# aws-samples/sample-s3-hybrid-cache

Hardware: AMD Instinct MI355X
Metric: LZ4 encode+decode GiB/s (device-resident), 64 KiB blocks, 1/2/4/8 GPU (higher is better)
Workload: dtype u8

## Files before the change

### sample-s3-hybrid-cache_amd/csrc/s3hc_kernels.hip

```cpp
#include <hip/hip_runtime.h>
#include <stdint.h>

#include "s3hc_plan.hpp"
#include "s3hc_knobs.hpp"
#include "s3hc_lz4.h"

namespace s3hc {

__device__ __forceinline__ uint32_t rotl32(uint32_t x, int r) {
    return __builtin_amdgcn_alignbit(x, x, 32 - r);
}
__device__ __forceinline__ uint32_t rdl(uint32_t v, uint32_t l) {
    return (uint32_t)__builtin_amdgcn_readlane((int)v, (int)l);
}
__device__ __forceinline__ int lane_id() { return __builtin_amdgcn_mbcnt_hi(~0u, __builtin_amdgcn_mbcnt_lo(~0u, 0)); }

#ifndef S3HC_WALK_PRIO
#define S3HC_WALK_PRIO 3
#endif
#define WALK_PRIO_ON() __builtin_amdgcn_s_setprio(S3HC_WALK_PRIO)
#define WALK_PRIO_OFF() __builtin_amdgcn_s_setprio(0)

__device__ __forceinline__ void wave_sync() {
    __builtin_amdgcn_fence(__ATOMIC_RELEASE, "wavefront");
    __builtin_amdgcn_wave_barrier();
    __builtin_amdgcn_fence(__ATOMIC_ACQUIRE, "wavefront");
}

#if defined(S3HC_DIAG_LEVEL) && S3HC_DIAG_LEVEL == 10
#define S3HC_PROF 1
__device__ unsigned long long g_prof[32];
#define PROF_NOW() __builtin_amdgcn_s_memtime()
#define PROF_ADD(arr, k, v) (arr)[k] += (v)
#else
#define PROF_NOW() 0ull
#define PROF_ADD(arr, k, v) ((void)(v))
#endif

__device__ __forceinline__ uint32_t lds32u(const uint8_t* lds, uint32_t i) {
    const uint32_t* w = (const uint32_t*)(lds + (i & ~3u));
    return __builtin_amdgcn_alignbyte(w[1], w[0], i & 3u);
}

__device__ __forceinline__ uint32_t gld32u(const uint8_t* p, uint32_t avail) {
    uintptr_t a = (uintptr_t)p;
    const uint32_t* w = (const uint32_t*)(a & ~(uintptr_t)3);
    uint32_t sh = (uint32_t)(a & 3);
    uint32_t lo = w[0];
    uint32_t hi = (sh != 0 && avail > 4 - sh) ? w[1] : 0u;
    return __builtin_amdgcn_alignbyte(hi, lo, sh);
}

template <int CTRL, int ROWMASK>
__device__ __forceinline__ uint32_t dpp0(uint32_t x) {
    return (uint32_t)__builtin_amdgcn_update_dpp(0, (int)x, CTRL, ROWMASK, 0xF, false);
}
__device__ __forceinline__ uint32_t wave_incl_sum(uint32_t x) {
    x += dpp0<0x111, 0xF>(x);
    x += dpp0<0x112, 0xF>(x);
    x += dpp0<0x114, 0xF>(x);
    x += dpp0<0x118, 0xF>(x);
    x += dpp0<0x142, 0xA>(x);
    x += dpp0<0x143, 0xC>(x);
    return x;
}
__device__ __forceinline__ uint32_t umax32(uint32_t a, uint32_t b) { return a > b ? a : b; }
__device__ __forceinline__ uint32_t umin32(uint32_t a, uint32_t b) { return a < b ? a : b; }
__device__ __forceinline__ uint32_t wave_incl_max(uint32_t x) {
    x = umax32(x, dpp0<0x111, 0xF>(x));
    x = umax32(x, dpp0<0x112, 0xF>(x));
    x = umax32(x, dpp0<0x114, 0xF>(x));
    x = umax32(x, dpp0<0x118, 0xF>(x));
    x = umax32(x, dpp0<0x142, 0xA>(x));
    x = umax32(x, dpp0<0x143, 0xC>(x));
    return x;
}
__device__ __forceinline__ uint32_t wave_excl_scan(uint32_t v, int) { return wave_incl_sum(v) - v; }
template <int CTRL, int ROWMASK>
__device__ __forceinline__ uint64_t dpp0_64(uint64_t x) {
    return (uint64_t)dpp0<CTRL, ROWMASK>((uint32_t)(x >> 32)) << 32 | dpp0<CTRL, ROWMASK>((uint32_t)x);
}
__device__ __forceinline__ uint64_t wave_incl_sum64(uint64_t x) {
    x += dpp0_64<0x111, 0xF>(x);
    x += dpp0_64<0x112, 0xF>(x);
    x += dpp0_64<0x114, 0xF>(x);
    x += dpp0_64<0x118, 0xF>(x);
    x += dpp0_64<0x142, 0xA>(x);
    x += dpp0_64<0x143, 0xC>(x);
    return x;
}

__device__ void wave_copy_global(uint8_t* dst, const uint8_t* src, uint32_t n, int lane) {
    uintptr_t da = (uintptr_t)dst;
    uint32_t head = (uint32_t)((16 - (da & 15)) & 15);
    if (head > n) head = n;
    if ((uint32_t)lane < head) dst[lane] = src[lane];
    const uint32_t nv = (n - head) >> 4;
    const uint8_t* s = src + head;
    uint8_t* d = dst + head;
    const uintptr_t sa = (uintptr_t)s;
    const uint32_t sh = (uint32_t)(sa & 3);
    const uint32_t* sw = (const uint32_t*)(sa & ~(uintptr_t)3);
    for (uint32_t base = 0; base < nv; base += 64 * 2) {
        const uint32_t ja = base + lane, jb = base + lane + 64;
        const uint32_t ka = ja < nv ? ja : nv - 1, kb = jb < nv ? jb : nv - 1;
        uint4 va, vb;
        if (sh == 0) {
            va = make_uint4(sw[4 * ka], sw[4 * ka + 1], sw[4 * ka + 2], sw[4 * ka + 3]);
            vb = make_uint4(sw[4 * kb], sw[4 * kb + 1], sw[4 * kb + 2], sw[4 * kb + 3]);
        } else {
            const uint32_t a0 = sw[4 * ka], a1 = sw[4 * ka + 1], a2 = sw[4 * ka + 2], a3 = sw[4 * ka + 3], a4 = sw[4 * ka + 4];
            const uint32_t b0 = sw[4 * kb], b1 = sw[4 * kb + 1], b2 = sw[4 * kb + 2], b3 = sw[4 * kb + 3], b4 = sw[4 * kb + 4];
            va = make_uint4(__builtin_amdgcn_alignbyte(a1, a0, sh), __builtin_amdgcn_alignbyte(a2, a1, sh),
                            __builtin_amdgcn_alignbyte(a3, a2, sh), __builtin_amdgcn_alignbyte(a4, a3, sh));
            vb = make_uint4(__builtin_amdgcn_alignbyte(b1, b0, sh), __builtin_amdgcn_alignbyte(b2, b1, sh),
                            __builtin_amdgcn_alignbyte(b3, b2, sh), __builtin_amdgcn_alignbyte(b4, b3, sh));
        }
        if (ja < nv) *(uint4*)(d + 16 * ja) = va;
        if (jb < nv) *(uint4*)(d + 16 * jb) = vb;
    }
    for (uint32_t t = head + 16 * nv + (uint32_t)lane; t < n; t += 64) dst[t] = src[t];
}

__device__ void wave_store_from_lds(uint8_t* dst, const uint8_t* lds, uint32_t n, int lane) {
    uintptr_t da = (uintptr_t)dst;
    uint32_t head = (uint32_t)((16 - (da & 15)) & 15);
    if (head > n) head = n;
    if ((uint32_t)lane < head) dst[lane] = lds[lane];
    uint32_t body = (n - head) & ~15u;
    for (uint32_t c = (uint32_t)lane * 16; c < body; c += 64 * 16) {
        uint32_t i = head + c;
        uint4 v = make_uint4(lds32u(lds, i), lds32u(lds, i + 4), lds32u(lds, i + 8), lds32u(lds, i + 12));
        *(uint4*)(dst + i) = v;
    }
    for (uint32_t t = head + body + (uint32_t)lane; t < n; t += 64) dst[t] = lds[t];
}

#define XP1 2654435761U
#define XP2 2246822519U
#define XP3 3266489917U
#define XP4 668265263U
#define XP5 374761393U

__device__ __forceinline__ uint32_t xround(uint32_t acc, uint32_t in) {
    acc += in * XP2;
    acc = rotl32(acc, 13);
    return acc * XP1;
}

template <uint32_t kIF, bool kPipe>
__device__ __forceinline__ uint32_t xxh32_lanes(const uint8_t* __restrict__ p, uint32_t L, bool act, uint32_t a) {
    const int lane = lane_id();
    const uint32_t ns = L >> 4;
    uint32_t acc = a == 0 ? XP1 + XP2 : (a == 1 ? XP2 : (a == 2 ? 0u : 0u - XP1));
    const uint8_t* q = p + 4 * a;
    uint32_t s = 0;
    if (kPipe && (((uintptr_t)p) & 3) == 0) {
        const uint32_t* w = (const uint32_t*)q;
        uint32_t b0[kIF], b1[kIF], b2[kIF];
        const uint32_t nbt = ns / kIF;
#define XLD(buf, bidx)                                                        \
    {                                                                         \
        const uint32_t bb_ = (bidx) < nbt ? (bidx) : 0u;                      \
        _Pragma("unroll") for (uint32_t k = 0; k < kIF; ++k) buf[k] = w[4 * (bb_ * kIF + k)]; \
    }
#define XUSE(buf) _Pragma("unroll") for (uint32_t k = 0; k < kIF; ++k) acc = xround(acc, buf[k]);
        XLD(b0, 0u)
        XLD(b1, 1u)
        for (uint32_t b = 0; b < nbt; b += 3) {
            XLD(b2, b + 2)
            XUSE(b0)
            XLD(b0, b + 3)
            if (b + 1 < nbt) { XUSE(b1) }
            XLD(b1, b + 4)
            if (b + 2 < nbt) { XUSE(b2) }
        }
#undef XLD
#undef XUSE
        for (s = nbt * kIF; s < ns; ++s) acc = xround(acc, w[4 * s]);
    } else if ((((uintptr_t)p) & 3) == 0) {
        const uint32_t* w = (const uint32_t*)q;
        for (; s + kIF <= ns; s += kIF) {
            uint32_t v[kIF];
#pragma unroll
            for (uint32_t k = 0; k < kIF; ++k) v[k] = w[4 * (s + k)];
#pragma unroll
            for (uint32_t k = 0; k < kIF; ++k) acc = xround(acc, v[k]);
        }
        for (; s < ns; ++s) acc = xround(acc, w[4 * s]);
// ... 1021 lines not shown
                    if (tll > limit - produced) st = S3HC_CORRUPT;
                    else if (tll > cap - produced) st = S3HC_DST_TOO_SMALL;
                    else if (tail == 1) {
                        const uint32_t have = produced + tll;
                        if (toff == 0 || toff > have + hist) st = S3HC_CORRUPT;
                        else if (tml > limit - have) st = S3HC_CORRUPT;
                        else if (tml > cap - have) st = S3HC_DST_TOO_SMALL;
                    }
                    if (st != S3HC_OK) { finish_block(st); continue; }
                    upos += tll + (tail == 1 ? tml : 0u);
                    blk_done = tail == 2;
                }
                if (n == 0 && tail == 0) {
                    if (blk_done) finish_block(S3HC_OK);
                    else q = cur;
                    continue;
                }
                cmd = dpe::C_WIN;
                emit_lo = n ? q + mis : 0xFFFFFFFFu;
                if (lane == 0) {
                    sl.S = S;
                    sl.n = n;
                    sl.ptr = (uint64_t)(uintptr_t)in;
                    sl.tail = tail;
                    sl.tlit = tlit;
                    sl.tll = tll;
                    sl.toff = toff;
                    sl.tml = tml;
                }
                if (blk_done) finish_block(S3HC_OK);
                else q = cur;
            }
            if (lane == 0) sl.cmd = cmd;
            prev_lo = emit_lo;
        } else if (it > 0) {
            const Slot& sl = slots[(it - 1u) & 1u];
            auto rfl = [](uint32_t v) -> uint32_t { return (uint32_t)__builtin_amdgcn_readfirstlane((int)v); };
            const uint32_t cmd = rfl(sl.cmd);
            const uint8_t* sptr = (const uint8_t*)(uintptr_t)(((uint64_t)rfl((uint32_t)(sl.ptr >> 32)) << 32) |
                                                              rfl((uint32_t)sl.ptr));
            if (cmd == dpe::C_WIN) {
                const uint32_t n = rfl(sl.n);
                if (n) {
                    const uint32_t a0 = w.upos & 3u;
                    const uint32_t r0 = (uint32_t)lane < n ? sl.orel[lane] : 0xFFFFu;
                    const uint32_t r1 = (uint32_t)lane + 64u < n ? sl.orel[64 + lane] : 0xFFFFu;
                    *(r0 != 0xFFFFu ? marks + r0 + a0 : sink + lane) = (uint8_t)(lane + 1);
                    *(r1 != 0xFFFFu ? marks + r1 + a0 : sink + lane) = (uint8_t)(lane + 65);
                    w.mtab = const_cast<uint2*>(sl.mtab);
                    wave_sync();
#ifndef S3HC_DIAG_NOEXEC
                    dec_window_passes(w, rfl(sl.S), rfl(sl.far) != 0u);
#else
                    w.upos += rfl(sl.S);
#endif
                }
                const uint32_t tail = rfl(sl.tail);
                if (tail) {
                    dec_literals(w, sptr, rfl(sl.tlit), rfl(sl.tll), 0xFFFFFFFFu, false);
                    if (tail == 1) dec_match(w, rfl(sl.toff), rfl(sl.tml));
                }
            } else if (cmd == dpe::C_STORED) {
                const uint32_t cs = rfl(sl.tlit);
                if (rfl(sl.single)) {
                    wave_copy_global(w.out, sptr, cs, lane);
                    w.upos = w.flushed = cs;
                } else {
                    dec_literals(w, sptr, 0, cs, 0xFFFFFFFFu, false);
                }
            } else if (cmd == dpe::C_END) {
                dec_final_flush(w);
                if (lane == 0) *done = 1u;
            }
        }
        __syncthreads();
        if (*done) break;
    }
}

__global__ __launch_bounds__(128) __attribute__((amdgpu_waves_per_eu(S3HC_PE_WAVES_PER_EU, 8))) void k_decode_pe(
    const uint8_t* __restrict__ src, uint8_t* dst, const DecBlock* __restrict__ blk, const DecUnit* __restrict__ units,
    uint32_t nunits, const uint64_t* __restrict__ ucount, uint32_t* __restrict__ blk_out,
    int32_t* __restrict__ blk_status, const uint8_t* __restrict__ unit_lb, const uint8_t* __restrict__ unit_fast) {
    __shared__ __attribute__((aligned(16))) uint8_t smem[dpe::kLds];
    const uint32_t nu = unit_count(ucount, nunits);
    for (uint32_t u = blockIdx.x; u < nu; u += gridDim.x) {
        decode_unit_pe(u, smem, src, dst, blk, units, blk_out, blk_status, unit_lb, unit_fast);
        __syncthreads();
    }
}

namespace enc {
constexpr uint32_t kPad = 16;
constexpr uint32_t kGIn = kPad + kPrewarm + kGroupSegs * kSeg + 128;
constexpr uint32_t kGThreads = 64 * kGroupSegs;
constexpr uint32_t kTbl = 1u << kHashLog;
#ifndef S3HC_STEPS
#define S3HC_STEPS 8
#endif
#ifndef S3HC_SHORT_GATE
#define S3HC_SHORT_GATE 1
#endif
#ifndef S3HC_LAZY
#define S3HC_LAZY 1
#endif
#ifndef S3HC_SALU_PAD
#define S3HC_SALU_PAD 0
#endif
#ifndef S3HC_VALU_PAD
#define S3HC_VALU_PAD 0
#endif
#ifndef S3HC_ABL
#define S3HC_ABL 0
#endif
#ifndef S3HC_ENC_MINWAVES
#define S3HC_ENC_MINWAVES 1
#endif
constexpr uint32_t kSteps = S3HC_STEPS;
constexpr uint32_t kStash = 64 * kSteps / 4;
#ifndef S3HC_FWD_DW
#define S3HC_FWD_DW 6
#endif
constexpr int kNQ = S3HC_FWD_DW;
constexpr uint32_t kFwd = 3 + 4 * kNQ;
constexpr uint32_t kEmpty = 0xFFFFu;
}

__device__ __forceinline__ uint32_t ext_bytes(uint32_t n) { return (n + 240u) / 255u; }
__device__ __forceinline__ uint32_t ffbl_hw(uint32_t x) {
    uint32_t r;
    asm("v_ffbl_b32 %0, %1" : "=v"(r) : "v"(x));
    return r;
}
__device__ __forceinline__ uint32_t ffbh_hw(uint32_t x) {
    uint32_t r;
    asm("v_ffbh_u32 %0, %1" : "=v"(r) : "v"(x));
    return r;
}
template <int N>
__device__ __forceinline__ uint32_t fwd_len(const uint32_t (&d)[N]) {
    uint32_t m = ffbl_hw(d[0]);
#pragma unroll
    for (int j = 1; j < N; ++j) m = umin32(m, __builtin_elementwise_add_sat(ffbl_hw(d[j]), 32u * (uint32_t)j));
    return (m >> 3) + 4u;
}
__device__ __forceinline__ uint32_t hash4(uint32_t v) { return (v * 2654435761u) >> (32 - kHashLog); }
__device__ __forceinline__ uint32_t hash_pos(uint32_t v, uint32_t b5) {
    return (b5 * 0x9E3779u + v * 2654435761u) >> (32 - kHashLog);
}

template <uint32_t kPSt>
__device__ __forceinline__ uint32_t next_landing(uint64_t mq, uint32_t np) {
    const uint32_t kk = (np + kPSt - 1u) / kPSt;
    const uint64_t rest = kk < 64u ? mq >> kk : 0ull;
    const uint32_t lo = (uint32_t)rest, hi = (uint32_t)(rest >> 32);
    const uint32_t tz = lo ? (uint32_t)__builtin_ctz(lo) : 32u + (uint32_t)__builtin_ctz(hi | 0x80000000u);
    return rest ? kk + tz : 64u;
}

__device__ void stage_in(const uint8_t* blk, uint32_t lo, uint32_t hi, uint8_t* lds, uint32_t lane, uint32_t nthr) {
    const uint32_t n = hi - lo;
    const uint8_t* g = blk + lo;
    const uint32_t nv = n >> 4;
    if (nv && (((uintptr_t)g) & 15) == 0) {
        const uint4* sv = (const uint4*)g;
        for (uint32_t base = 0; base < nv; base += nthr * 8) {
            uint4 v0, v1, v2, v3, v4, v5, v6, v7;
#define S3HC_LD(q, vq) { const uint32_t j = base + lane + nthr * q; vq = sv[j < nv ? j : nv - 1]; }
            S3HC_LD(0, v0) S3HC_LD(1, v1) S3HC_LD(2, v2) S3HC_LD(3, v3)
            S3HC_LD(4, v4) S3HC_LD(5, v5) S3HC_LD(6, v6) S3HC_LD(7, v7)
#undef S3HC_LD
#define S3HC_ST(q, vq) { const uint32_t j = base + lane + nthr * q; if (j < nv) *(uint4*)(lds + 16 * j) = vq; }
            S3HC_ST(0, v0) S3HC_ST(1, v1) S3HC_ST(2, v2) S3HC_ST(3, v3)
            S3HC_ST(4, v4) S3HC_ST(5, v5) S3HC_ST(6, v6) S3HC_ST(7, v7)
#undef S3HC_ST
        }
    } else if (nv) {
        const uintptr_t a = (uintptr_t)g & ~(uintptr_t)3;
        const uint32_t sh = (uint32_t)((uintptr_t)g & 3);
        const uint32_t* sw = (const uint32_t*)a;
        for (uint32_t base = 0; base < nv; base += nthr * 2) {
            const uint32_t ja = base + lane, jb = base + lane + nthr;
            const uint32_t ka = ja < nv ? ja : nv - 1, kb = jb < nv ? jb : nv - 1;
            const uint32_t a0 = sw[4 * ka], a1 = sw[4 * ka + 1], a2 = sw[4 * ka + 2], a3 = sw[4 * ka + 3];
            const uint32_t a4 = sh ? sw[4 * ka + 4] : 0u;
            const uint32_t b0 = sw[4 * kb], b1 = sw[4 * kb + 1], b2 = sw[4 * kb + 2], b3 = sw[4 * kb + 3];
            const uint32_t b4 = sh ? sw[4 * kb + 4] : 0u;
            if (ja < nv)
                *(uint4*)(lds + 16 * ja) = make_uint4(__builtin_amdgcn_alignbyte(a1, a0, sh), __builtin_amdgcn_alignbyte(a2, a1, sh),
                                                      __builtin_amdgcn_alignbyte(a3, a2, sh), __builtin_amdgcn_alignbyte(a4, a3, sh));
            if (jb < nv)
                *(uint4*)(lds + 16 * jb) = make_uint4(__builtin_amdgcn_alignbyte(b1, b0, sh), __builtin_amdgcn_alignbyte(b2, b1, sh),
                                                      __builtin_amdgcn_alignbyte(b3, b2, sh), __builtin_amdgcn_alignbyte(b4, b3, sh));
        }
    }
    for (uint32_t t = 16 * nv + lane; t < n; t += nthr) lds[t] = g[t];
}

#ifdef S3HC_ENC_WPE
#define S3HC_ENC_WPE_ATTR __attribute__((amdgpu_num_vgpr(512 / S3HC_ENC_WPE / 8 * 8)))
#else
#define S3HC_ENC_WPE_ATTR
#endif
template <uint32_t kPS, uint32_t kIns>
__global__ __launch_bounds__(enc::kGThreads, S3HC_ENC_MINWAVES) S3HC_ENC_WPE_ATTR void k_enc_parse(const uint8_t* __restrict__ src,
                                                              const EncBlock* __restrict__ blocks,
                                                              const uint2* __restrict__ groups, uint32_t ngroups,
                                                              uint32_t nxx, const uint64_t* __restrict__ fsrc_off,
                                                              const uint32_t* __restrict__ fsrc_len, uint32_t nframes,
                                                              uint32_t* __restrict__ fhash, uint2* __restrict__ recs,
                                                              SegSummary* __restrict__ summ) {
    using namespace enc;
    static_assert(kPS == 1 || kPS == 2, "probe stride 1 or 2");
    constexpr uint32_t kStepPos = 64 * kPS;
    constexpr uint32_t kPSteps = kSteps / kPS;
    __shared__ __attribute__((aligned(16))) uint8_t inb_raw[kGIn];
    __shared__ __attribute__((aligned(16))) uint16_t tbl_all[kGroupSegs][kTbl + 8];
    __shared__ __attribute__((aligned(16))) uint2 stash_all[kGroupSegs][kStash + 8];
#ifdef S3HC_ENC_LDS_PAD
    __shared__ uint8_t enc_pad[S3HC_ENC_LDS_PAD];
    if (ngroups == 0xFFFFFFFFu) ((volatile uint8_t*)enc_pad)[threadIdx.x] = 0;
#endif
    if (blockIdx.x < nxx) {
#ifndef S3HC_ENC_NOXXH
        xxh32_ranges_dev<32, false>(src, fsrc_off, fsrc_len, nframes, fhash, blockIdx.x * kGThreads + threadIdx.x);
#endif
        return;
    }
    const uint32_t gi = blockIdx.x - nxx;
    if (gi >= ngroups) return;
    const uint2 G = groups[gi];
    const EncBlock B = blocks[G.x];
    const uint32_t U = B.len;
    const uint32_t ns = B.nseg - G.y < kGroupSegs ? B.nseg - G.y : kGroupSegs;
    const uint32_t g_lo = G.y * kSeg;
    const uint32_t g_hi = g_lo + ns * kSeg < U ? g_lo + ns * kSeg : U;
    const uint32_t stage_lo = g_lo > kPrewarm ? g_lo - kPrewarm : 0;
    const uint32_t stage_hi = g_hi + 64 < U ? g_hi + 64 : U;
    const uint8_t* bin = src + B.src_off;
    const uint32_t wv = (uint32_t)__builtin_amdgcn_readfirstlane((int)(threadIdx.x >> 6));
    const int lane = lane_id();
    uint16_t* tbl = tbl_all[wv];
    uint2* stash = stash_all[wv];
    for (uint32_t t = lane; t < (kTbl + 8) / 8; t += 64) ((uint4*)tbl)[t] = make_uint4(~0u, ~0u, ~0u, ~0u);
    stage_in(bin, stage_lo, stage_hi, inb_raw + kPad, threadIdx.x, kGThreads);
    __syncthreads();
    if (wv >= ns) return;
#ifdef S3HC_PROF
    uint64_t epr[9] = {0, 0, 0, 0, 0, 0, 0, 0, 0};
    const uint64_t tk0 = PROF_NOW();
#endif
    const uint32_t k = G.y + wv;
    const uint32_t s = B.seg0 + k;
    const uint32_t seg_lo = k * kSeg;
    const uint32_t seg_hi = seg_lo + kSeg < U ? seg_lo + kSeg : U;
    const uint32_t pw_lo = seg_lo > kPrewarm ? seg_lo - kPrewarm : 0;
    uint8_t* inb = inb_raw + kPad + (pw_lo - stage_lo);
    const uint32_t* dw = (const uint32_t*)inb;
    const uint32_t ia_max = kGIn - kPad - (pw_lo - stage_lo) - 8;
    const uint32_t blk_end_lim = U >= 5 ? U - 5 : 0;
    const uint32_t end_lim = seg_hi < blk_end_lim ? seg_hi : blk_end_lim;
    int64_t smax = (int64_t)end_lim - 4;
    if ((int64_t)U - 12 < smax) smax = (int64_t)U - 12;
    {
        const uint32_t lim = seg_lo - pw_lo;
        for (uint32_t d0 = lane; 4 * d0 < lim; d0 += 64) {
            const uint32_t w0 = dw[d0], w1 = dw[d0 + 1];
#pragma unroll
            for (uint32_t j = 0; j < 4; ++j) {
                const uint32_t i = 4 * d0 + j;
                tbl[i + 4 <= lim ? hash_pos(__builtin_amdgcn_alignbyte(w1, w0, j), __builtin_amdgcn_ubfe(w1, 8 * j, 8)) : kTbl] = (uint16_t)i;
            }
        }
    }
    wave_sync();
#ifdef S3HC_PROF
    epr[0] = PROF_NOW() - tk0;
#endif
    uint32_t x = seg_lo;
    uint32_t last_end = seg_lo;
    uint32_t nseq = 0, body = 0, ll0 = 0;
    uint2* myrec = recs + (size_t)s * kMaxSeqPerSeg;
    const uint32_t pend = smax < (int64_t)seg_lo ? seg_lo : (uint32_t)(smax + 1);
    for (uint32_t sb = seg_lo; sb < pend; sb += 64 * kSteps) {
        const uint32_t sb_end = sb + 64 * kSteps < pend ? sb + 64 * kSteps : pend;
        const uint64_t tc0 = PROF_NOW();
        PROF_ADD(epr, 6, 1);
        uint32_t vv[kPSteps], vm[kPSteps], vm8[kPSteps], cc[kPSteps];
#pragma unroll
        for (uint32_t q = 0; q < kPSteps; ++q) {
            const uint32_t P = sb + kStepPos * q + kPS * lane;
            const uint32_t i = P - pw_lo;
            const uint32_t a = i >> 2, sh = i & 3;
            const uint32_t w0 = dw[a], w1 = dw[a + 1], wp = dw[(int)a - 1], wpp = dw[(int)a - 2];
            vv[q] = __builtin_amdgcn_alignbyte(w1, w0, sh);
            vm[q] = __builtin_amdgcn_alignbyte(w0, wp, sh);
            vm8[q] = __builtin_amdgcn_alignbyte(wp, wpp, sh);
            const uint32_t h = hash_pos(vv[q], __builtin_amdgcn_ubfe(w1, 8 * sh, 8));
            if (kPS == 1) {
                cc[q] = tbl[h];
                if constexpr (kIns != 0) {
                    if ((P < sb_end) & ((P & kIns) == 0)) tbl[h] = (uint16_t)i;
                } else {
                    tbl[P < sb_end ? h : kTbl] = (uint16_t)i;
                }
            } else {
                const uint32_t h1 = hash_pos(__builtin_amdgcn_alignbyte(w1, w0, sh + 1), __builtin_amdgcn_ubfe(w1, 8 * (sh + 1), 8));
                const uint32_t t0 = P < sb_end ? h : kTbl, t1 = P + 1 < sb_end ? h1 : kTbl;
#pragma unroll
                for (uint32_t half = 0; half < 2; ++half) {
                    if (((uint32_t)lane >> 5) == half) {
                        cc[q] = tbl[h];
                        tbl[t0] = (uint16_t)i;
                        tbl[t1] = (uint16_t)(i + 1);
                    }
                    wave_sync();
                }
            }
        }
        uint32_t word[kPSteps], flen[kPSteps];
        uint64_t mm[kPSteps];
#pragma unroll
        for (uint32_t q = 0; q < kPSteps; ++q) {
            const uint32_t P = sb + kStepPos * q + kPS * lane;
            const bool valid = P < sb_end;
            const uint32_t i = P - pw_lo;
            const uint32_t v = vv[q], vm4 = vm[q];
            const bool e1 = __builtin_amdgcn_alignbyte(v, vm4, 3) == v, e2 = __builtin_amdgcn_alignbyte(v, vm4, 2) == v;
            const bool e3 = __builtin_amdgcn_alignbyte(v, vm4, 1) == v, e4 = vm4 == v;
#ifndef S3HC_SHORT_CAND
#define S3HC_SHORT_CAND 1
#endif
            const uint32_t c16 = cc[q];
#if S3HC_SHORT_CAND == 2
            const uint32_t dfs = (e1 & (i >= 5u)) ? 1u : ((e2 & (i >= 6u)) ? 2u : ((e3 & (i >= 7u)) ? 3u : ((e4 & (i >= 8u)) ? 4u : 0u)));
            const bool per = (dfs != 0u) & (__builtin_amdgcn_alignbyte(vm4, vm8[q], (4u - dfs) & 3u) == vm4);
            const bool tin = per | ((c16 != kEmpty) & (c16 < i));
            const uint32_t ct = per ? i - dfs : (tin ? c16 : i);
#else
            const bool tin = (c16 != kEmpty) & (c16 < i);
            const uint32_t ct = tin ? c16 : i;
#endif
            const uint32_t a = i >> 2, sh = i & 3, ta = ct >> 2, ts = ct & 3;
            uint32_t O[kNQ + 1], T[kNQ + 3];
#pragma unroll
            for (int j = 0; j < kNQ + 1; ++j) O[j] = dw[a + 1 + j];
#pragma unroll
            for (int j = 0; j < kNQ + 3; ++j) T[j] = dw[(int)ta - 1 + j];
            uint32_t Q[kNQ + 1];
            Q[0] = v;
#pragma unroll
            for (int j = 0; j < kNQ; ++j) Q[j + 1] = __builtin_amdgcn_alignbyte(O[j + 1], O[j], sh);
            const uint32_t maxf = end_lim - P;
            uint32_t dtt[kNQ];
#pragma unroll
            for (int j = 0; j < kNQ; ++j) dtt[j] = Q[j + 1] ^ __builtin_amdgcn_alignbyte(T[j + 3], T[j + 2], ts);
            uint32_t lt = umin32(umin32(fwd_len(dtt), kFwd), maxf);
            const uint32_t bt = vm4 ^ __builtin_amdgcn_alignbyte(T[1], T[0], ts);
            const uint32_t nbt = umin32(umin32(ffbh_hw(bt) >> 3, 4u), ct);
            const bool gt = valid & tin & (__builtin_amdgcn_alignbyte(T[2], T[1], ts) == v);
            uint32_t len = lt, nb = nbt, dist = i - ct;
            bool gf = false;
#ifndef S3HC_SHORT_MIN
#define S3HC_SHORT_MIN 24
#endif
#if S3HC_SHORT_GATE
            bool want_short = valid & (e1 | e2 | e3 | e4) & !gt;
#else
            bool want_short = valid & (e1 | e2 | e3 | e4) & !(gt & (lt >= S3HC_SHORT_MIN));
#endif
#if S3HC_ABL == 2
            want_short = false;
#endif
            if (S3HC_SHORT_CAND == 1 && __ballot(want_short)) {
                const uint32_t df = (e1 & (i >= 1)) ? 1u : ((e2 & (i >= 2)) ? 2u : ((e3 & (i >= 3)) ? 3u : ((e4 & (i >= 4)) ? 4u : 0u)));
                gf = want_short & (df != 0);
                const uint32_t fs = (4u - df) & 3u;
                uint32_t dff[kNQ];
#pragma unroll
                for (int j = 0; j < kNQ; ++j) dff[j] = Q[j + 1] ^ __builtin_amdgcn_alignbyte(Q[j + 1], Q[j], fs);
                const uint32_t lf = umin32(umin32(fwd_len(dff), kFwd), maxf);
                const uint32_t bf = vm4 ^ __builtin_amdgcn_alignbyte(vm4, vm8[q], fs);
                const uint32_t nbf = umin32(umin32(ffbh_hw(bf) >> 3, 4u), i - df);
                const bool ut = gt & (!gf | (lt >= lf));
                len = ut ? lt : lf;
                nb = ut ? nbt : nbf;
                dist = ut ? i - ct : df;
            }
            word[q] = dist | ((len - 4) << 16) | (nb << 24);
            flen[q] = len;
#if S3HC_LAZY
            const uint32_t fv = (gt | gf) ? len : 0u;
            const uint32_t fnext = (uint32_t)__builtin_amdgcn_update_dpp(0, (int)fv, 0x130, 0xF, 0xF, false);
            mm[q] = __ballot((gt | gf) & !((fnext > fv) & (fv < kFwd)));
#else
            mm[q] = __ballot(gt | gf);
#endif
#if S3HC_SALU_PAD
            {
                uint32_t d0 = q;
#pragma unroll
                for (int k = 0; k < S3HC_SALU_PAD; ++k) asm volatile("s_add_u32 %0, %0, 1" : "+s"(d0));
                asm volatile("" ::"s"(d0));
            }
#endif
#if S3HC_VALU_PAD
            {
                uint32_t d1 = lane;
#pragma unroll
                for (int k = 0; k < S3HC_VALU_PAD; ++k) asm volatile("v_add_u32 %0, %0, 1" : "+v"(d1));
                asm volatile("" ::"v"(d1));
            }
#endif
            if (q & 1) wave_sync();
        }
        const uint64_t tc1 = PROF_NOW();
        PROF_ADD(epr, 1, tc1 - tc0);
        const uint32_t ns_sb = nseq, le_sb = last_end;
        WALK_PRIO_ON();
#pragma unroll
        for (uint32_t q = 0; q < kPSteps; ++q) {
            const uint32_t base = sb + kStepPos * q;
            if (x >= base + kStepPos || !mm[q]) continue;
            uint64_t hm = 0;
            const uint64_t mq = mm[q];
            const uint32_t np = kPS * (uint32_t)lane + flen[q];
            const uint32_t nl = next_landing<kPS>(mq, np);
            const uint32_t nxl = flen[q] == kFwd ? 0x80u : (nl < 64u ? nl : 0x100u | np);
            uint32_t r = x > base ? x - base : 0u;
            uint32_t j0 = (r + kPS - 1u) / kPS;
            uint64_t av = j0 < 64u ? mq & (~0ull << j0) : 0ull;
#if S3HC_ABL == 1
            hm = mq & 0x1111111111111111ull;
            r = kStepPos;
            av = 0;
#endif
            while (av) {
                uint32_t j = (uint32_t)__builtin_ctzll(av);
                uint32_t v;
                for (;;) {
                    hm |= 1ull << j;
                    v = rdl(nxl, j);
                    if (v >= 64u) break;
                    j = v;
                }
                if (v & 0x100u) {
                    r = v & 0xFFu;
                    break;
                }
                {
                    const uint64_t tx0 = PROF_NOW();
                    PROF_ADD(epr, 8, 1);
                    const uint32_t wj = rdl(word[q], j);
                    const uint32_t P = base + kPS * j;
                    const uint32_t maxf = end_lim - P;
                    const uint32_t c = P - (wj & 0xFFFFu);
                    uint32_t lenf = kFwd;
                    while (lenf < maxf) {
                        const uint32_t rel = lenf + 4u * lane;
                        uint32_t e2;
                        if (rel >= maxf) {
                            e2 = 0;
                        } else {
                            uint32_t ia = P + rel - pw_lo;
                            if (ia > ia_max) ia = ia_max;
                            const uint32_t xa = lds32u(inb, ia), ya = lds32u(inb, c + rel - pw_lo);
                            e2 = xa == ya ? 4u : (uint32_t)__builtin_ctz(xa ^ ya) >> 3;
                            if (e2 > maxf - rel) e2 = maxf - rel;
                        }
                        const uint64_t m2 = __ballot(e2 != 4u);
                        if (m2 == 0) { lenf += 256; continue; }
                        const uint32_t g = (uint32_t)__builtin_ctzll(m2);
                        lenf += 4u * g + rdl(e2, g);
                        break;
                    }
                    flen[q] = (uint32_t)lane == j ? lenf : flen[q];
                    r = kPS * j + lenf;
                    PROF_ADD(epr, 2, PROF_NOW() - tx0);
                }
                j0 = (r + kPS - 1u) / kPS;
                av = j0 < 64u ? mq & (~0ull << j0) : 0ull;
            }
            x = base + r;
            if (hm) {
                const uint32_t rank =
                    __builtin_amdgcn_mbcnt_hi((uint32_t)(hm >> 32), __builtin_amdgcn_mbcnt_lo((uint32_t)hm, 0));
                const uint32_t hidx = (hm >> lane) & 1ull ? nseq - ns_sb + rank : kStash + ((uint32_t)lane & 7u);
                stash[hidx] = make_uint2((base + kPS * lane - seg_lo) | (flen[q] << 16), word[q]);
                last_end = base + r;
                nseq += (uint32_t)__builtin_popcountll(hm);
            }
        }
        WALK_PRIO_OFF();
        const uint64_t tf0 = PROF_NOW();
        wave_sync();
        {
#if S3HC_ABL == 4
            const uint32_t H = 0;
            body += stash[lane].x + stash[lane].y;
#else
            const uint32_t H = nseq - ns_sb;
#endif
            uint32_t carry_end = le_sb;
            for (uint32_t g = 0; g < H; g += 64) {
                const uint32_t idx = g + lane;
                const bool act = idx < H;
                const uint2 e = stash[act ? idx : 0u];
                const uint32_t P = seg_lo + (e.x & 0xFFFFu), lenf = e.x >> 16, wd = e.y;
                const uint32_t endj = P + lenf;
                const uint32_t pe = dpp0<0x138, 0xF>(endj);
                const uint32_t prev = lane == 0 ? carry_end : pe;
                uint32_t nb = (wd >> 24) & 7u;
                nb = nb > P - prev ? P - prev : nb;
                const uint32_t ll = P - nb - prev;
                const uint32_t len = nb + lenf;
                const uint32_t gj = ns_sb + idx;
                const uint32_t tok = gj == 0 ? 0u : 1u + ext_bytes(ll);
                const uint32_t sz = act ? tok + ll + 2u + ext_bytes(len - 4) : 0u;
                body += rdl(wave_incl_sum(sz), 63);
                if (ns_sb == 0 && g == 0) ll0 = rdl(ll, 0);
                if (act) myrec[gj] = make_uint2(ll | (len << 16), wd & 0xFFFFu);
                const uint32_t last = H - g < 64 ? H - g - 1 : 63u;
                carry_end = rdl(endj, last);
            }
        }
        wave_sync();
        PROF_ADD(epr, 4, PROF_NOW() - tf0);
        PROF_ADD(epr, 3, PROF_NOW() - tc1);
    }
#ifdef S3HC_PROF
    epr[5] = PROF_NOW() - tk0;
    epr[7] = nseq;
    if (lane == 0)
        for (int q = 0; q < 9; ++q) atomicAdd(&g_prof[16 + q], (unsigned long long)epr[q]);
#endif
    if (lane == 0) {
        SegSummary S;
#if S3HC_ABL == 1 || S3HC_ABL == 4
        nseq = 0;
#endif
        S.nseq = nseq;
        S.ll0 = ll0;
        S.body = body;
        S.trail = seg_hi - last_end;
        summ[s] = S;
    }
}

__global__ void k_enc_sizes(const EncBlock* __restrict__ blocks, uint32_t nblocks,
                            const SegSummary* __restrict__ summ, SegPlace* __restrict__ place,
                            uint32_t* __restrict__ blk_payload, uint32_t* __restrict__ blk_size,
                            uint32_t* __restrict__ blk_carry) {
    const uint32_t b = blockIdx.x * blockDim.x + threadIdx.x;
    if (b >= nblocks) return;
    const EncBlock B = blocks[b];
    const uint32_t hdr = (B.flags & EB_FIRST) ? 7u : 0u;
    const uint32_t trl = (B.flags & EB_LAST) ? 8u : 0u;
    if (B.flags & EB_EMPTY) {
        blk_payload[b] = 0;
        blk_size[b] = hdr + trl;
        blk_carry[b] = 0;
        return;
    }
    uint32_t payload = B.len;
    bool stored = true;
    uint32_t carry = 0;
    if (!(B.flags & EB_STORE)) {
        uint32_t off = 0;
        for (uint32_t k = 0; k < B.nseg; ++k) {
            const SegSummary S = summ[B.seg0 + k];
            const uint32_t lo = k * kSeg;
            const uint32_t hi = lo + kSeg < B.len ? lo + kSeg : B.len;
            SegPlace P;
            P.out_off = off;
            P.carry = carry;
            place[B.seg0 + k] = P;
            if (S.nseq == 0) {
                carry += hi - lo;
                continue;
            }
            const uint32_t lle = carry + S.ll0;
            off += 1 + ext_bytes(lle) + carry + S.body;
            carry = S.trail;
        }
        off += 1 + ext_bytes(carry) + carry;
        if (off < B.len) {
            stored = false;
            payload = off;
        }
    }
    blk_payload[b] = payload | (stored ? kStoredBit : 0u);
    blk_size[b] = hdr + 4 + payload + trl;
    blk_carry[b] = carry;
}

__global__ __launch_bounds__(256) void k_enc_emit(const uint8_t* __restrict__ src,
                                                  const EncBlock* __restrict__ blocks,
                                                  const uint32_t* __restrict__ seg_block, uint32_t nseg,
                                                  const uint2* __restrict__ recs,
                                                  const SegSummary* __restrict__ summ,
                                                  const SegPlace* __restrict__ place,
                                                  const uint32_t* __restrict__ blk_payload,
                                                  const uint32_t* __restrict__ blk_carry,
                                                  const uint64_t* __restrict__ blk_off,
                                                  const uint32_t* __restrict__ frame_hash, uint8_t* dst) {
    constexpr uint32_t kOut = kSeg + 256;
    constexpr uint32_t kIb = kSeg + 64;
    constexpr uint32_t kWaveLds = kOut + kIb;
    __shared__ __attribute__((aligned(16))) uint8_t smem[2 * kWaveLds];
    const int lane = lane_id();
    const uint32_t wv = (uint32_t)__builtin_amdgcn_readfirstlane((int)(threadIdx.x >> 6));
    const uint32_t s = blockIdx.x * 2 + wv;
    if (s >= nseg) return;
    uint8_t* ob = smem + wv * kWaveLds;
    uint8_t* ib = ob + kOut;
    const uint32_t b = seg_block[s];
    const EncBlock B = blocks[b];
    const uint32_t k = s - B.seg0;
    uint8_t* fo = dst + blk_off[b];
    const uint32_t hdr = (B.flags & EB_FIRST) ? 7u : 0u;
    const uint32_t pw = blk_payload[b];
    const bool stored = (pw & kStoredBit) != 0;
    const uint32_t payload = pw & ~kStoredBit;
    const uint32_t fh = frame_hash[B.frame];
    if (k == 0 && lane == 0) {
        if (B.flags & EB_FIRST) {
            fo[0] = 0x04; fo[1] = 0x22; fo[2] = 0x4D; fo[3] = 0x18;
            fo[4] = kFlgIndependentChecksum; fo[5] = B.bd; fo[6] = B.hc;
        }
        if (!(B.flags & EB_EMPTY)) {
            const uint32_t word = stored ? (B.len | kStoredBit) : payload;
            fo[hdr + 0] = (uint8_t)word; fo[hdr + 1] = (uint8_t)(word >> 8);
            fo[hdr + 2] = (uint8_t)(word >> 16); fo[hdr + 3] = (uint8_t)(word >> 24);
        }
    }
    const bool last_seg = k + 1 == B.nseg;
    if ((B.flags & EB_LAST) && last_seg && lane < 8) {
        const uint32_t tpos = (B.flags & EB_EMPTY) ? hdr : hdr + 4 + payload;
        const uint32_t v = lane < 4 ? 0u : fh;
        fo[tpos + lane] = (uint8_t)(v >> (8 * (lane & 3)));
    }
    if (B.flags & EB_EMPTY) return;
    uint8_t* pay = fo + hdr + 4;
    const uint32_t seg_lo = k * kSeg;
    const uint32_t seg_hi = seg_lo + kSeg < B.len ? seg_lo + kSeg : B.len;
    const uint8_t* bin = src + B.src_off;
    if (stored) {
        wave_copy_global(pay + seg_lo, bin + seg_lo, seg_hi - seg_lo, lane);
        return;
    }
    const SegSummary S = summ[s];
    const SegPlace P = place[s];
    uint32_t o = P.out_off;
    if (S.nseq > 0) {
        const uint2* rr = recs + (size_t)s * kMaxSeqPerSeg;
        auto ldr = [&](uint32_t k) -> uint2 {
            const uint32_t jk = 64u * k + (uint32_t)lane;
            return rr[jk < S.nseq ? jk : 0u];
        };
        const uint2 pre0 = ldr(0), pre1 = ldr(1), pre2 = ldr(2), pre3 = ldr(3);
        const uint32_t ml0 = rdl(pre0.x, 0) >> 16;
        const uint32_t lle = P.carry + S.ll0;
        const uint32_t ne = ext_bytes(lle);
        if (lane == 0) {
            const uint32_t mn = ml0 - 4;
            pay[o] = (uint8_t)(((lle < 15 ? lle : 15) << 4) | (mn < 15 ? mn : 15));
        }
        for (uint32_t e = lane; e < ne; e += 64) pay[o + 1 + e] = e + 1 < ne ? 255 : (uint8_t)((lle - 15) % 255);
        o += 1 + ne;
        wave_copy_global(pay + o, bin + seg_lo - P.carry, P.carry, lane);
        o += P.carry;
        stage_in(bin, seg_lo, seg_hi, ib, lane, 64);
        wave_sync();
        uint32_t ob_len = 0;
        uint32_t in_pos = 0;
        for (uint32_t g = 0; g < S.nseq; g += 64) {
            const uint32_t j = g + lane;
            const bool act = j < S.nseq;
            uint2 r = g == 0 ? pre0 : (g == 64 ? pre1 : (g == 128 ? pre2 : pre3));
            if (g >= 256u) r = act ? rr[j] : make_uint2(0, 0);
            if (!act) r = make_uint2(0, 0);
            const uint32_t ll = r.x & 0xFFFFu, ml = r.x >> 16, off = r.y;
            const uint32_t hsz = j == 0 ? 0u : 1 + ext_bytes(ll);
            const uint32_t sz = act ? hsz + ll + 2 + ext_bytes(ml - 4) : 0u;
            const uint32_t opos = ob_len + wave_excl_scan(sz, lane);
            const uint32_t ipos = in_pos + wave_excl_scan(act ? ll + ml : 0u, lane);
            const uint32_t tot = rdl(opos + sz, 63) - ob_len;
// ... 310 lines not shown
    if (got_hash) got_hash[f] = h;
    if (st == S3HC_OK) {
        const uint8_t* fp = src + frame_off[f];
        const uint32_t flg = fp[4];
        if ((flg & 0x08) && (rd32(fp + 6) | ((uint64_t)rd32(fp + 10) << 32)) != L) st = S3HC_CORRUPT;
        else if ((flg & 0x04) && !defer && h != fwant[f]) st = S3HC_CHECKSUM;
    }
    if (pend) pend[f] = defer && st == S3HC_OK ? 1u : 0u;
    fstatus[f] = st;
}
__global__ __launch_bounds__(64) void k_dframe_close(const uint8_t* __restrict__ src, const uint64_t* __restrict__ frame_off,
                                                     const uint64_t* __restrict__ blk_base, const uint32_t* __restrict__ nblk,
                                                     const DecBlock* __restrict__ blocks, const uint32_t* __restrict__ blk_out,
                                                     const int32_t* __restrict__ blk_status,
                                                     const uint64_t* __restrict__ blk_hash, const uint8_t* __restrict__ out,
                                                     const uint64_t* __restrict__ out_off, const uint32_t* __restrict__ fwant,
                                                     uint32_t n, const int32_t* fstat_in, int32_t* fstatus,
                                                     uint32_t* __restrict__ out_len, uint32_t* __restrict__ got_hash,
                                                     uint32_t* __restrict__ pend) {
    dframe_close_lane(blockIdx.x * blockDim.x + threadIdx.x, src, frame_off, blk_base, nblk, blocks, blk_out, blk_status,
                      blk_hash, out, out_off, fwant, n, fstat_in, fstatus, out_len, got_hash, pend);
}

}

namespace s3hc {
static inline uint32_t cdiv(uint64_t a, uint64_t b) { return (uint32_t)((a + b - 1) / b); }

hipError_t launch_xxh32(const uint8_t* base, const uint64_t* off, const uint32_t* len, uint32_t n, uint32_t* out,
                        hipStream_t st) {
    if (!n) return hipSuccess;
    hipLaunchKernelGGL(k_xxh32_ranges, dim3(cdiv((uint64_t)n * 4, 64)), dim3(64), 0, st, base, off, len, n, out);
    return hipGetLastError();
}
hipError_t launch_decode_units(const uint8_t* src, uint8_t* dst, const DecBlock* blk, const DecUnit* units,
                               uint32_t nunits, const uint64_t* ucount, uint32_t grid, uint32_t* blk_out,
                               int32_t* blk_status, const uint8_t* unit_lb, const uint8_t* unit_fast, hipStream_t st) {
    if (!nunits || !grid) return hipSuccess;
#if S3HC_DIAG_VARIANTS
    if (knob_on(KN_DEC_ONEWAVE)) {
        hipLaunchKernelGGL(k_decode_units, dim3(cdiv(grid, dec::kWaves)), dim3(64 * dec::kWaves), 0, st, src, dst,
                           blk, units, nunits, ucount, blk_out, blk_status, unit_lb, unit_fast);
        return hipGetLastError();
    }
#endif
    hipLaunchKernelGGL(k_decode_pe, dim3(grid), dim3(128), 0, st, src, dst, blk, units, nunits, ucount, blk_out,
                       blk_status, unit_lb, unit_fast);
    return hipGetLastError();
}
hipError_t launch_enc_parse(const uint8_t* src, const EncBlock* blocks, const uint2* groups, uint32_t ngroups,
                            const uint64_t* fsrc_off, const uint32_t* fsrc_len, uint32_t nframes, uint32_t* fhash,
                            uint2* recs, SegSummary* summ, int mode, hipStream_t st) {
    const uint32_t nxx = cdiv((uint64_t)nframes * 4, enc::kGThreads);
    if (!ngroups && !nxx) return hipSuccess;
    if (mode == 1)
        hipLaunchKernelGGL((k_enc_parse<1, 1>), dim3(nxx + ngroups), dim3(enc::kGThreads), 0, st, src, blocks, groups,
                           ngroups, nxx, fsrc_off, fsrc_len, nframes, fhash, recs, summ);
    else
        hipLaunchKernelGGL((k_enc_parse<2, 0>), dim3(nxx + ngroups), dim3(enc::kGThreads), 0, st, src, blocks, groups,
                           ngroups, nxx, fsrc_off, fsrc_len, nframes, fhash, recs, summ);
    return hipGetLastError();
}
hipError_t launch_enc_sizes(const EncBlock* blocks, uint32_t nblocks, const SegSummary* summ, SegPlace* place,
                            uint32_t* blk_payload, uint32_t* blk_size, uint32_t* blk_carry, hipStream_t st) {
    if (!nblocks) return hipSuccess;
    hipLaunchKernelGGL(k_enc_sizes, dim3(cdiv(nblocks, 256)), dim3(256), 0, st, blocks, nblocks, summ, place,
                       blk_payload, blk_size, blk_carry);
    return hipGetLastError();
}
hipError_t launch_scan(const uint32_t* in, uint32_t n, uint64_t* out, uint64_t* total, hipStream_t st) {
    hipLaunchKernelGGL(k_scan_u32_u64, dim3(1), dim3(1024), 0, st, in, n, out, total);
    return hipGetLastError();
}
hipError_t launch_scan2(const uint32_t* in0, const uint32_t* in1, uint32_t n, uint64_t* out0, uint64_t* out1,
                        uint64_t* total, hipStream_t st) {
    hipLaunchKernelGGL(k_scan2_u32_u64, dim3(2), dim3(1024), 0, st, in0, in1, n, out0, out1, total);
    return hipGetLastError();
}
hipError_t launch_enc_emit(const uint8_t* src, const EncBlock* blocks, const uint32_t* seg_block, uint32_t nseg,
                           const uint2* recs, const SegSummary* summ, const SegPlace* place,
                           const uint32_t* blk_payload, const uint32_t* blk_carry, const uint64_t* blk_off,
                           const uint32_t* frame_hash, uint8_t* dst, hipStream_t st) {
    if (!nseg) return hipSuccess;
    hipLaunchKernelGGL(k_enc_emit, dim3(cdiv(nseg, 2)), dim3(128), 0, st, src, blocks, seg_block, nseg, recs, summ,
                       place, blk_payload, blk_carry, blk_off, frame_hash, dst);
    return hipGetLastError();
}
hipError_t launch_enc_groups(const uint32_t* g_blk0, const uint32_t* g_nblk, uint32_t ng, const uint64_t* blk_off,
                             const uint32_t* blk_size, uint64_t* g_off, uint32_t* g_len, hipStream_t st) {
    if (!ng) return hipSuccess;
    hipLaunchKernelGGL(k_enc_frames, dim3(cdiv(ng, 256)), dim3(256), 0, st, g_blk0, g_nblk, ng, blk_off, blk_size,
                       g_off, g_len);
    return hipGetLastError();
}
hipError_t launch_dframe_count(const uint8_t* src, const uint64_t* frame_off, const uint32_t* frame_len,
                               const uint32_t* dst_cap, uint32_t n, uint32_t* nblk, int32_t* fstatus,
                               hipStream_t st) {
    if (!n) return hipSuccess;
    hipLaunchKernelGGL(k_dframe_count, dim3(cdiv(n, 256)), dim3(256), 0, st, src, frame_off, frame_len, dst_cap, n,
                       nblk, fstatus);
    return hipGetLastError();
}
hipError_t launch_dframe_fill(const uint8_t* src, const uint64_t* frame_off, const uint32_t* frame_len, uint32_t n,
                              const uint64_t* dst_off, const uint32_t* dst_cap, const uint64_t* blk_base,
                              const int32_t* fstatus, DecBlock* blocks, DecUnit* units, uint32_t* fwant,
                              const uint64_t* ftok, hipStream_t st) {
    if (!n) return hipSuccess;
    hipLaunchKernelGGL(k_dframe_fill, dim3(cdiv(n, 256)), dim3(256), 0, st, src, frame_off, frame_len, n, dst_off,
                       dst_cap, blk_base, fstatus, blocks, units, fwant, ftok);
    return hipGetLastError();
}
hipError_t launch_dframe_finish(const uint64_t* blk_base, uint32_t n, const uint32_t* nblk, const DecBlock* blocks,
                                const uint32_t* blk_out, const int32_t* blk_status, int32_t* fstatus,
                                uint32_t* out_len, hipStream_t st) {
    if (!n) return hipSuccess;
    hipLaunchKernelGGL(k_dframe_finish, dim3(cdiv(n, 256)), dim3(256), 0, st, blk_base, n, nblk, blocks, blk_out,
                       blk_status, fstatus, out_len);
    return hipGetLastError();
}
hipError_t launch_dframe_close(const uint8_t* src, const uint64_t* frame_off, const uint64_t* blk_base,
                               const uint32_t* nblk, const DecBlock* blocks, const uint32_t* blk_out,
                               const int32_t* blk_status, const uint64_t* blk_hash, const uint8_t* out,
                               const uint64_t* out_off, const uint32_t* fwant, uint32_t n, const int32_t* fstat_in,
                               int32_t* fstatus, uint32_t* out_len, uint32_t* got_hash, hipStream_t st,
                               uint32_t* pend) {
    if (!n) return hipSuccess;
    hipLaunchKernelGGL(k_dframe_close, dim3(cdiv((uint64_t)n * kCloseLanes, 64)), dim3(64), 0, st, src, frame_off, blk_base, nblk,
                       blocks, blk_out, blk_status, blk_hash, out, out_off, fwant, n, fstat_in, fstatus, out_len,
                       got_hash, pend);
    return hipGetLastError();
}
hipError_t launch_dframe_verify(const uint8_t* src, const uint64_t* frame_off, uint32_t n, const uint32_t* fwant,
                                const uint32_t* got, const uint32_t* out_len, int32_t* fstatus, hipStream_t st) {
    if (!n) return hipSuccess;
    hipLaunchKernelGGL(k_dframe_verify, dim3(cdiv(n, 256)), dim3(256), 0, st, src, frame_off, n, fwant, got, out_len,
                       fstatus);
    return hipGetLastError();
}
}

#ifdef S3HC_PROF
extern "C" int s3hc_diag_prof(unsigned long long* out, int n, int reset) {
    if (n > 32) n = 32;
    if (hipDeviceSynchronize() != hipSuccess) return -1;
    if (hipMemcpyFromSymbol(out, HIP_SYMBOL(s3hc::g_prof), sizeof(unsigned long long) * n) != hipSuccess) return -1;
    if (reset) {
        unsigned long long z[32] = {0};
        if (hipMemcpyToSymbol(HIP_SYMBOL(s3hc::g_prof), z, sizeof(z)) != hipSuccess) return -1;
    }
    return 0;
}
#endif

#include "s3hc_fast.hip"
```

Before: 161.1.

## Micro-optimize LZ4 encoder walk: branchless landing, writelane, hoisted addressing, prewarm pipelining

Several small encoder-kernel tweaks land together. next_landing now uses hardware find-first-bit with saturating adds instead of branches. The per-lane forward length is updated with v_writelane instead of a lane-compare select. Word-address and shift computation are hoisted out of the per-step loops. The prewarm hash-table fill is rewritten as a software-pipelined fixed-trip loop. A compile-time-gated event counter diagnostic is also added, and it is inactive by default.

```diff
diff --git a/sample-s3-hybrid-cache_amd/csrc/s3hc_kernels.hip b/sample-s3-hybrid-cache_amd/csrc/s3hc_kernels.hip
--- a/sample-s3-hybrid-cache_amd/csrc/s3hc_kernels.hip
+++ b/sample-s3-hybrid-cache_amd/csrc/s3hc_kernels.hip
@@ -12,6 +12,9 @@
 }
 __device__ __forceinline__ uint32_t rdl(uint32_t v, uint32_t l) {
     return (uint32_t)__builtin_amdgcn_readlane((int)v, (int)l);
+}
+__device__ __forceinline__ void wrl(uint32_t& v, uint32_t x, uint32_t l) {
+    asm("s_mov_b32 m0, %2\n\tv_writelane_b32 %0, %1, m0" : "+v"(v) : "s"(x), "s"(l) : "m0");
 }
 __device__ __forceinline__ int lane_id() { return __builtin_amdgcn_mbcnt_hi(~0u, __builtin_amdgcn_mbcnt_lo(~0u, 0)); }
 
@@ -35,6 +38,13 @@
 #else
 #define PROF_NOW() 0ull
 #define PROF_ADD(arr, k, v) ((void)(v))
+#endif
+#if defined(S3HC_DIAG_LEVEL) && S3HC_DIAG_LEVEL == 11
+#define S3HC_ENC_COUNT 1
+__device__ unsigned long long g_enc_cnt[16];
+#define CNT_ADD(k, v) ecn[k] += (v)
+#else
+#define CNT_ADD(k, v) ((void)0)
 #endif
 
 __device__ __forceinline__ uint32_t lds32u(const uint8_t* lds, uint32_t i) {
@@ -1362,10 +1372,9 @@
 template <uint32_t kPSt>
 __device__ __forceinline__ uint32_t next_landing(uint64_t mq, uint32_t np) {
     const uint32_t kk = (np + kPSt - 1u) / kPSt;
-    const uint64_t rest = kk < 64u ? mq >> kk : 0ull;
-    const uint32_t lo = (uint32_t)rest, hi = (uint32_t)(rest >> 32);
-    const uint32_t tz = lo ? (uint32_t)__builtin_ctz(lo) : 32u + (uint32_t)__builtin_ctz(hi | 0x80000000u);
-    return rest ? kk + tz : 64u;
+    const uint64_t rest = mq >> (kk & 63u);
+    const uint32_t tz = umin32(ffbl_hw((uint32_t)rest), __builtin_elementwise_add_sat(ffbl_hw((uint32_t)(rest >> 32)), 32u));
+    return __builtin_elementwise_add_sat(kk, tz);
 }
 
 __device__ void stage_in(const uint8_t* blk, uint32_t lo, uint32_t hi, uint8_t* lds, uint32_t lane, uint32_t nthr) {
@@ -1460,6 +1469,9 @@
     uint64_t epr[9] = {0, 0, 0, 0, 0, 0, 0, 0, 0};
     const uint64_t tk0 = PROF_NOW();
 #endif
+#ifdef S3HC_ENC_COUNT
+    uint32_t ecn[14] = {1, 0, 0, 0, 0, 0, 0, 0, 0, 0, 0, 0, 0, 0};
+#endif
     const uint32_t k = G.y + wv;
     const uint32_t s = B.seg0 + k;
     const uint32_t seg_lo = k * kSeg;
@@ -1472,16 +1484,23 @@
     const uint32_t end_lim = seg_hi < blk_end_lim ? seg_hi : blk_end_lim;
     int64_t smax = (int64_t)end_lim - 4;
     if ((int64_t)U - 12 < smax) smax = (int64_t)U - 12;
-    {
-        const uint32_t lim = seg_lo - pw_lo;
-        for (uint32_t d0 = lane; 4 * d0 < lim; d0 += 64) {
-            const uint32_t w0 = dw[d0], w1 = dw[d0 + 1];
+    static_assert(kPrewarm <= kSeg && kPrewarm % 256 == 0, "the prewarm window is whole or absent");
+    if (seg_lo != pw_lo) {
+        auto put = [&](uint32_t w0, uint32_t w1, uint32_t d0, auto last) {
 #pragma unroll
             for (uint32_t j = 0; j < 4; ++j) {
                 const uint32_t i = 4 * d0 + j;
-                tbl[i + 4 <= lim ? hash_pos(__builtin_amdgcn_alignbyte(w1, w0, j), __builtin_amdgcn_ubfe(w1, 8 * j, 8)) : kTbl] = (uint16_t)i;
-            }
-        }
+                const uint32_t h = hash_pos(j ? __builtin_amdgcn_alignbyte(w1, w0, j) : w0, __builtin_amdgcn_ubfe(w1, 8 * j, 8));
+                tbl[(!decltype(last)::value || j == 0 || i + 4 <= kPrewarm) ? h : kTbl] = (uint16_t)i;
+            }
+        };
+        uint32_t d0 = lane, w0 = dw[d0], w1 = dw[d0 + 1];
+        for (uint32_t it = 0; it + 1 < kPrewarm / 256; ++it) {
+            const uint32_t n0 = dw[d0 + 64], n1 = dw[d0 + 65];
+            put(w0, w1, d0, std::false_type{});
+            w0 = n0, w1 = n1, d0 += 64;
+        }
+        put(w0, w1, d0, std::true_type{});
     }
     wave_sync();
 #ifdef S3HC_PROF
@@ -1491,9 +1510,11 @@
     uint32_t last_end = seg_lo;
     uint32_t nseq = 0, body = 0, ll0 = 0;
     uint2* myrec = recs + (size_t)s * kMaxSeqPerSeg;
+    const uint32_t sh = (kPS * (uint32_t)lane) & 3u, la = (kPS * (uint32_t)lane) >> 2;
     const uint32_t pend = smax < (int64_t)seg_lo ? seg_lo : (uint32_t)(smax + 1);
     for (uint32_t sb = seg_lo; sb < pend; sb += 64 * kSteps) {
         const uint32_t sb_end = sb + 64 * kSteps < pend ? sb + 64 * kSteps : pend;
+        const uint32_t sa = (sb - pw_lo) >> 2;
         const uint64_t tc0 = PROF_NOW();
         PROF_ADD(epr, 6, 1);
         uint32_t vv[kPSteps], vm[kPSteps], vm8[kPSteps], cc[kPSteps];
@@ -1501,7 +1522,7 @@
         for (uint32_t q = 0; q < kPSteps; ++q) {
             const uint32_t P = sb + kStepPos * q + kPS * lane;
             const uint32_t i = P - pw_lo;
-            const uint32_t a = i >> 2, sh = i & 3;
+            const uint32_t a = sa + la + kStepPos / 4 * q;
             const uint32_t w0 = dw[a], w1 = dw[a + 1], wp = dw[(int)a - 1], wpp = dw[(int)a - 2];
             vv[q] = __builtin_amdgcn_alignbyte(w1, w0, sh);
             vm[q] = __builtin_amdgcn_alignbyte(w0, wp, sh);
@@ -1551,7 +1572,7 @@
             const bool tin = (c16 != kEmpty) & (c16 < i);
             const uint32_t ct = tin ? c16 : i;
 #endif
-            const uint32_t a = i >> 2, sh = i & 3, ta = ct >> 2, ts = ct & 3;
+            const uint32_t a = sa + la + kStepPos / 4 * q, ta = ct >> 2, ts = ct & 3;
             uint32_t O[kNQ + 1], T[kNQ + 3];
 #pragma unroll
             for (int j = 0; j < kNQ + 1; ++j) O[j] = dw[a + 1 + j];
@@ -1582,7 +1603,14 @@
 #if S3HC_ABL == 2
             want_short = false;
 #endif
+            CNT_ADD(1, __ballot(valid) ? 1u : 0u);
             if (S3HC_SHORT_CAND == 1 && __ballot(want_short)) {
+#ifdef S3HC_ENC_COUNT
+                const uint32_t wpc = (uint32_t)__builtin_popcountll(__ballot(want_short));
+                CNT_ADD(2, 1);
+                CNT_ADD(3 + (wpc <= 3 ? wpc - 1 : (wpc < 8 ? 3 : (wpc < 16 ? 4 : (wpc < 32 ? 5 : 6)))), 1);
+                CNT_ADD(10, wpc);
+#endif
                 const uint32_t df = (e1 & (i >= 1)) ? 1u : ((e2 & (i >= 2)) ? 2u : ((e3 & (i >= 3)) ? 3u : ((e4 & (i >= 4)) ? 4u : 0u)));
                 gf = want_short & (df != 0);
                 const uint32_t fs = (4u - df) & 3u;
@@ -1634,10 +1662,13 @@
             if (x >= base + kStepPos || !mm[q]) continue;
             uint64_t hm = 0;
             const uint64_t mq = mm[q];
-            const uint32_t np = kPS * (uint32_t)lane + flen[q];
+            uint32_t fl = flen[q];
+            uint32_t np = kPS * (uint32_t)lane + fl;
+            asm("" : "+v"(np));
             const uint32_t nl = next_landing<kPS>(mq, np);
-            const uint32_t nxl = flen[q] == kFwd ? 0x80u : (nl < 64u ? nl : 0x100u | np);
-            uint32_t r = x > base ? x - base : 0u;
+            const uint32_t nxl = fl == kFwd ? 0x80u : (nl < 64u ? nl : 0x100u | np);
+            const int32_t xr = (int32_t)(x - base);
+            uint32_t r = (uint32_t)(xr > 0 ? xr : 0);
             uint32_t j0 = (r + kPS - 1u) / kPS;
             uint64_t av = j0 < 64u ? mq & (~0ull << j0) : 0ull;
 #if S3HC_ABL == 1
@@ -1648,7 +1679,9 @@
             while (av) {
                 uint32_t j = (uint32_t)__builtin_ctzll(av);
                 uint32_t v;
+                CNT_ADD(11, 1);
                 for (;;) {
+                    CNT_ADD(12, 1);
                     hm |= 1ull << j;
                     v = rdl(nxl, j);
                     if (v >= 64u) break;
@@ -1661,6 +1694,7 @@
                 {
                     const uint64_t tx0 = PROF_NOW();
                     PROF_ADD(epr, 8, 1);
+                    CNT_ADD(13, 1);
                     const uint32_t wj = rdl(word[q], j);
                     const uint32_t P = base + kPS * j;
                     const uint32_t maxf = end_lim - P;
@@ -1684,7 +1718,7 @@
                         lenf += 4u * g + rdl(e2, g);
                         break;
                     }
-                    flen[q] = (uint32_t)lane == j ? lenf : flen[q];
+                    wrl(fl, lenf, j);
                     r = kPS * j + lenf;
                     PROF_ADD(epr, 2, PROF_NOW() - tx0);
                 }
@@ -1696,7 +1730,7 @@
                 const uint32_t rank =
                     __builtin_amdgcn_mbcnt_hi((uint32_t)(hm >> 32), __builtin_amdgcn_mbcnt_lo((uint32_t)hm, 0));
                 const uint32_t hidx = (hm >> lane) & 1ull ? nseq - ns_sb + rank : kStash + ((uint32_t)lane & 7u);
-                stash[hidx] = make_uint2((base + kPS * lane - seg_lo) | (flen[q] << 16), word[q]);
+                stash[hidx] = make_uint2((base + kPS * lane - seg_lo) | (fl << 16), word[q]);
                 last_end = base + r;
                 nseq += (uint32_t)__builtin_popcountll(hm);
             }
@@ -1743,6 +1777,10 @@
     epr[7] = nseq;
     if (lane == 0)
         for (int q = 0; q < 9; ++q) atomicAdd(&g_prof[16 + q], (unsigned long long)epr[q]);
+#endif
+#ifdef S3HC_ENC_COUNT
+    if (lane == 0)
+        for (int q = 0; q < 14; ++q) atomicAdd(&g_enc_cnt[q], (unsigned long long)ecn[q]);
 #endif
     if (lane == 0) {
         SegSummary S;
@@ -2359,4 +2397,17 @@
 }
 #endif
 
+#ifdef S3HC_ENC_COUNT
+extern "C" int s3hc_diag_enc_counts(unsigned long long* out, int n, int reset) {
+    if (n > 16) n = 16;
+    if (hipDeviceSynchronize() != hipSuccess) return -1;
+    if (hipMemcpyFromSymbol(out, HIP_SYMBOL(s3hc::g_enc_cnt), sizeof(unsigned long long) * n) != hipSuccess) return -1;
+    if (reset) {
+        unsigned long long z[16] = {0};
+        if (hipMemcpyToSymbol(HIP_SYMBOL(s3hc::g_enc_cnt), z, sizeof(z)) != hipSuccess) return -1;
+    }
+    return 0;
+}
+#endif
+
 #include "s3hc_fast.hip"
```

Result: faster. 169.5 (median of 6 runs) (+5.2%).
